# wizardyesterday/RtlSdrDiags

Hardware: NVIDIA B200
Metric: aggregate_iq_msamples_per_s (higher is better)
Workload: dtype q15 int32 + f32

## Files before the change

### rtlsdrdiags_b200/csrc/sdr_device.cuh

```cuda
#pragma once
#include "sdr_platform.h"
#include "sdr_q15_taps.h"

namespace sdr {

enum { FMT_U8_OFFSET_ROTATE = 0, FMT_S8_ROTATED = 1 };
enum { MODE_NONE = 0, MODE_AM = 1, MODE_FM = 2, MODE_WBFM = 3, MODE_LSB = 4, MODE_USB = 5 };

constexpr int MAX_G = 32;
constexpr int FM_LUT_MIN = -140;
constexpr int FM_LUT_DIM = 280;

struct LaunchParams {
  const uint8_t *iq;
  uint64_t ch_stride;
  uint32_t n_samples;
  int fmt;
  const uint32_t *chan_ids;
  uint32_t n_list;
  uint32_t G;
  uint8_t *state;
  uint32_t state_stride;
  const float *scale;
  const uint8_t *lsb;
// ... 2 lines not shown
  const float *lut;
  uint32_t aux;
  int16_t *scratch;
  const uint8_t *allowed;
  uint32_t call_id;
  const uint32_t *tab;
  unsigned long long *trace;
  uint32_t seg_count, seg_rows, warm_rows;
  uint32_t *counters;
};

#if SDR_DEVICE_BUILD
__device__ __forceinline__ unsigned long long trace_now() {
  unsigned long long t;
  asm volatile("mov.u64 %0, %%globaltimer;" : "=l"(t));
  return t;
}
__device__ __forceinline__ void trace_begin(const LaunchParams &p) {
  if (p.trace && threadIdx.x == 0) atomicMin(p.trace, trace_now());
}
__device__ __forceinline__ void trace_end(const LaunchParams &p) {
  if (p.trace && threadIdx.x == 0) atomicMax(p.trace + 1, trace_now());
}
#endif

SDR_DEV int f2i16_wrap(float v) {
  int r = f2i_rz(v);
  if (!(fabsf(v) < 2147483648.0f)) r = 0;
  return (int)(int16_t)(uint16_t)(uint32_t)r;
}

SDR_DEV float wrap_pi(float d) {
  const float PI_F = 3.14159274101257324f;
  const double off = d >= PI_F ? -6.283185307179586 : (d <= -PI_F ? 6.283185307179586 : 0.0);
  return dadd_to_f(d, off);
}

SDR_DEV float wrap_pi_table(float d) {
  const float PI_F = 3.14159274101257324f;
  const float sgn = u2f((f2u(d) & 0x80000000u) | 0x3F800000u);
  const float w = ffma(sgn, u2f(0x343BBD2Eu) ,
                       ffma(sgn, u2f(0xC0C90FDBu) , d));
  return fabsf(d) >= PI_F ? w : d;
}

SDR_DEV uint32_t offset_and_negate(uint32_t raw, uint32_t neg, uint32_t one) {
// ... 203 lines not shown
```

### rtlsdrdiags_b200/csrc/sdr_engine.cu

```cuda
#include <cuda.h>
#include <cuda_runtime.h>
#include <math.h>
#include <stdio.h>
#include <stdlib.h>
#include <string.h>

#include <algorithm>
#include <string>
#include <vector>

#include "../../include/sdr_b200.h"
#include "sdr_config.h"

namespace {

using namespace sdr;

thread_local std::string g_create_error;

struct Shape { uint32_t G = 0, NT = 0; };

}

struct sdr_engine {
  int device = 0;
  uint32_t n = 0;
  uint64_t max_bytes = 0;
  int n_sm = 148;
  int smem_optin = 227 * 1024;
  cudaStream_t own_stream = nullptr, stream = nullptr;
  cudaStream_t rec_stream = nullptr;
  static constexpr int RING_MAX = 3;
  static constexpr int ring = RING_MAX;
  cudaEvent_t ev_fir[RING_MAX] = {}, ev_rec[RING_MAX] = {};
  static constexpr int RUN_AHEAD = 32, PACE = 2 * RUN_AHEAD;
  cudaEvent_t ev_pace[PACE] = {};
  int16_t *d_scratch[5][RING_MAX] = {};
  int tile_loader = 2;
  bool stage1_mma = false;
  int wb_kernel = 0;
  volatile uint32_t *h_wb_clip = nullptr;
  uint32_t wb_clip_seen = 0;
  uint64_t wb4_units = 0;
  int wb_clip_hold = 0;
  int wb4_geometry = 0;
  bool wb_count = false;
  bool wb_prefilter_mma = false;
  int fir_ctas_per_sm = 5;
  uint32_t *d_am_tab = nullptr;
  CUtensorMap tmap;
  const void *tmap_iq = nullptr;
  uint64_t tmap_stride = 0, tmap_rows = 0;
  uint32_t dc_seg_count = 0, dc_warm_rows = 28;
  uint32_t *d_counters = nullptr;
  uint64_t seq = 0;
  bool rec_pending = false;
  cudaStream_t wb_stream = nullptr;
  cudaEvent_t ev_in = nullptr, ev_wb = nullptr;
  bool wb_pending = false;
  int scaling = SDR_SCALING_RADIODIAGS;

  std::vector<uint8_t> mode, lsb;
  std::vector<float> gain[5], scale[5];
  std::vector<uint32_t> list[5];
  bool lists_dirty = true, lsb_dirty = true, scale_dirty[5] = {true, true, true, true, true};

  uint8_t *d_state[5] = {};
  float *d_scale[5] = {};
  uint32_t *d_list[5] = {};
  uint8_t *d_lsb = nullptr;
  float *d_lut_fm = nullptr, *d_lut_wbfm = nullptr;
  float *d_lut_wbfm_half = nullptr;
  uint32_t *d_fm_tab = nullptr;
  uint32_t *d_wb_tab = nullptr;
  uint8_t *d_wb4_tab = nullptr;
  uint8_t *d_iq = nullptr;
  int16_t *d_pcm2[2] = {nullptr, nullptr};
  uint64_t pcm_stride = 0;
  int16_t *pcm_of(uint64_t call) const { return d_pcm2[call & 1]; }
// ... 62 lines not shown
  }
  return 0;
}

float default_gain(int kind, int scaling) {
  switch (kind) {
    case SDR_KIND_AM: return 300;
    case SDR_KIND_FM: return (float)(64000 / (2 * M_PI));
    case SDR_KIND_WBFM:
      return scaling == SDR_SCALING_RESEARCH ? (float)(64000 / (2 * M_PI)) : (float)(256000 / (2 * M_PI));
    case SDR_KIND_SSB: return 300;
  }
  return 0;
}

float scale_of(int kind, float gain, int scaling) {
  if (kind == SDR_KIND_AM || kind == SDR_KIND_SSB || scaling == SDR_SCALING_RESEARCH) return gain;
  volatile float k = gain / (kind == SDR_KIND_FM ? 15000.0f : 75000.0f);
  k = k * 32767.0f;
  return k;
}

int join_streams(sdr_engine *e) {
  if (e->rec_pending) {
    SDR_CK(e, cudaStreamWaitEvent(e->stream, e->ev_rec[(e->seq + (uint64_t)e->ring - 1) % (uint64_t)e->ring], 0));
    e->rec_pending = false;
  }
  if (e->wb_pending) {
    SDR_CK(e, cudaStreamWaitEvent(e->stream, e->ev_wb, 0));
    e->wb_pending = false;
  }
  return SDR_OK;
}

typedef CUresult (*TensorMapEncodeTiled)(CUtensorMap *, CUtensorMapDataType, cuuint32_t, void *, const cuuint64_t *,
                                         const cuuint64_t *, const cuuint32_t *, const cuuint32_t *,
                                         CUtensorMapInterleave, CUtensorMapSwizzle, CUtensorMapL2promotion,
                                         CUtensorMapFloatOOBfill);
int iq_tensor_map(sdr_engine *e, const uint8_t *iq, uint64_t ch_stride, uint32_t n_samples) {
  const uint64_t rows = (uint64_t)(n_samples / TILE) * (TILE_BYTES / 128);
  if (e->tmap_iq == iq && e->tmap_stride == ch_stride && e->tmap_rows == rows) return SDR_OK;
  static TensorMapEncodeTiled encode = nullptr;
  if (!encode) {
    void *fn = nullptr;
    cudaDriverEntryPointQueryResult qr;
    SDR_CK(e, cudaGetDriverEntryPoint("cuTensorMapEncodeTiled", &fn, cudaEnableDefault, &qr));
    if (!fn || qr != cudaDriverEntryPointSuccess) return fail(e, SDR_E_CUDA, "the driver has no cuTensorMapEncodeTiled");
    encode = (TensorMapEncodeTiled)fn;
  }
  if (rows == 0) {
// ... 45 lines not shown
    };
    for (int lane = 0; lane < 32; ++lane) {
      const int g = lane >> 2, tq = lane & 3;
      uint32_t *t = tab.data() + ((size_t)f * 32 + lane) * 12;
      for (int h = 0; h < 2; ++h)
        for (int s2 = 0; s2 < 2; ++s2)
          for (int r = 0; r < 2; ++r) {
            const int k0 = 32 * s2 + 16 * r + 4 * tq;
            uint32_t w = 0;
            for (int b = 0; b < 4; ++b) w |= (uint32_t)(uint8_t)(int8_t)part(B[k0 + b][g], h) << (8 * b);
            t[(h * 2 + s2) * 2 + r] = w;
          }
      for (int i = 0; i < 4; ++i) {
        const int h = i >> 1, col = 2 * tq + (i & 1);
        int sum = 0;
        for (int kb = 0; kb < 64; ++kb) sum += part(B[kb][col], h);
        t[8 + i] = (uint32_t)((h == 1 ? 1 << 15 : 0) - (f == 0 ? 128 * sum : 0));
      }
    }
  }
  return tab;
}

template <bool SSB>
int launch_amssb(sdr_engine *e, int kind, const uint8_t *iq, uint64_t ch_stride, uint32_t n_samples, int fmt) {
  using T = AmSsbTile<SSB>;
  const uint32_t n_list = (uint32_t)e->list[kind].size();
  if (n_list == 0) return SDR_OK;
  const int par = (int)(e->seq % (uint64_t)e->ring);
  const uint32_t n_tiles = (n_samples + TILE - 1) / TILE;
  if (!e->d_scratch[kind][par]) {
    const size_t max_tiles = (size_t)((e->max_bytes / 2 + TILE - 1) / TILE);
    for (int i = 0; i < e->ring; ++i)
      if (!e->d_scratch[kind][i])
        SDR_CK(e, cudaMalloc(&e->d_scratch[kind][i], (size_t)e->n * max_tiles * 32 * sizeof(int16_t)));
  }
  static const int wps_env = getenv("SDR_AM_WARPS_PER_SM") ? atoi(getenv("SDR_AM_WARPS_PER_SM")) : 0;
  const uint64_t total_tiles = (uint64_t)n_list * n_tiles;
  uint64_t n_warps = (uint64_t)e->n_sm * (wps_env > 0 ? wps_env : (SSB ? 48 : 72));
  static const int min_share_env = getenv("SDR_AM_MIN_SHARE") ? atoi(getenv("SDR_AM_MIN_SHARE")) : 0;
  const uint64_t min_share = min_share_env > 0 ? (uint64_t)min_share_env : 16;
  n_warps = std::min<uint64_t>(n_warps, (total_tiles + min_share - 1) / min_share);
  n_warps = std::max<uint64_t>(n_warps, 1);
  LaunchParams p = {};
  p.iq = iq;
  p.ch_stride = ch_stride;
  p.n_samples = n_samples;
  p.fmt = fmt;
  p.chan_ids = e->d_list[kind];
  p.n_list = n_list;
  p.G = 4;
  p.state = e->d_state[kind];
  p.state_stride = (uint32_t)T::STATE_BYTES;
  p.scale = e->d_scale[kind];
  p.lsb = e->d_lsb;
  p.pcm = e->pcm_of(e->seq);
  p.pcm_stride = e->pcm_stride;
  p.lut = nullptr;
  p.aux = (uint32_t)n_warps;
  p.call_id = (uint32_t)(e->seq % 0x7fffffffull) + 1;
  p.scratch = e->d_scratch[kind][par];
  p.allowed = e->last_gated ? e->d_allowed[par] : nullptr;
  p.trace = e->d_trace ? e->d_trace + 4 * (e->seq % sdr_engine::TRACE_CALLS) : nullptr;
  const uint32_t grid = (uint32_t)((n_warps + 3) / 4);
  if (e->tile_loader == 0) {
    if (e->fir_ctas_per_sm == 6) amssb_fir_kernel<SSB, false, 2, false, 6><<<grid, 128, 4 * 2 * TILE_BYTES, e->stream>>>(p, e->tmap);
    else amssb_fir_kernel<SSB, false, 2, false><<<grid, 128, 4 * 2 * TILE_BYTES, e->stream>>>(p, e->tmap);
  } else if (e->fir_ctas_per_sm == 6 && !e->stage1_mma) {
    const int rc = iq_tensor_map(e, iq, ch_stride, n_samples);
    if (rc) return rc;
    if (e->tile_loader == 2) amssb_fir_kernel<SSB, true, 2, false, 6><<<grid, 128, 4 * 2 * TILE_BYTES, e->stream>>>(p, e->tmap);
    else amssb_fir_kernel<SSB, true, 4, false, 6><<<grid, 128, 4 * 4 * TILE_BYTES, e->stream>>>(p, e->tmap);
  } else {
    int rc = iq_tensor_map(e, iq, ch_stride, n_samples);
    if (rc) return rc;
    if (e->stage1_mma && !e->d_am_tab) {
      const std::vector<uint32_t> tab = am_mma_table();
      SDR_CK(e, cudaMalloc(&e->d_am_tab, tab.size() * 4));
      SDR_CK(e, cudaMemcpy(e->d_am_tab, tab.data(), tab.size() * 4, cudaMemcpyHostToDevice));
    }
    p.tab = e->d_am_tab;
    const int nst = e->tile_loader;
    const size_t smem = (size_t)4 * nst * TILE_BYTES;
    if (e->stage1_mma) {
      if (nst == 2) amssb_fir_kernel<SSB, true, 2, true><<<grid, 128, smem, e->stream>>>(p, e->tmap);
      else if (nst == 3) amssb_fir_kernel<SSB, true, 3, true><<<grid, 128, smem, e->stream>>>(p, e->tmap);
      else amssb_fir_kernel<SSB, true, 4, true><<<grid, 128, smem, e->stream>>>(p, e->tmap);
    } else {
      if (nst == 2) amssb_fir_kernel<SSB, true, 2, false><<<grid, 128, smem, e->stream>>>(p, e->tmap);
      else if (nst == 3) amssb_fir_kernel<SSB, true, 3, false><<<grid, 128, smem, e->stream>>>(p, e->tmap);
      else amssb_fir_kernel<SSB, true, 4, false><<<grid, 128, smem, e->stream>>>(p, e->tmap);
    }
  }
  SDR_CK(e, cudaGetLastError());
  e->launches++;
  return SDR_OK;
}

void dc_segments(const sdr_engine *e, uint32_t n_rows, uint32_t *seg_count, uint32_t *seg_rows) {
  uint32_t S = 1;
  if (e->dc_seg_count) {
    S = e->dc_seg_count;
  } else if (n_rows >= 64) {
    while (S < 32 && n_rows / (2 * S) >= 32) S *= 2;
  }
  while (S > 1 && (n_rows + S - 1) / S * (S - 1) >= n_rows) S /= 2;
  *seg_count = S;
  *seg_rows = (n_rows + S - 1) / S;
}

int launch_dc_block(sdr_engine *e, int kind, uint32_t n_samples) {
  const uint32_t n_list = (uint32_t)e->list[kind].size();
  if (n_list == 0) return SDR_OK;
  const int par = (int)(e->seq % (uint64_t)e->ring);
  const int nreg = kind == SDR_KIND_SSB ? AmSsbTile<true>::NREG : AmSsbTile<false>::NREG;
  LaunchParams p = {};
  p.n_samples = n_samples;
  p.chan_ids = e->d_list[kind];
  p.n_list = n_list;
  p.state = e->d_state[kind];
  p.state_stride = (uint32_t)state_bytes(kind);
  p.scale = e->d_scale[kind];
  p.pcm = e->pcm_of(e->seq);
  p.pcm_stride = e->pcm_stride;
  p.aux = (uint32_t)nreg * 256;
  p.scratch = e->d_scratch[kind][par];
  p.allowed = e->last_gated ? e->d_allowed[par] : nullptr;
  p.trace = e->d_trace ? e->d_trace + 4 * (e->seq % sdr_engine::TRACE_CALLS) + 2 : nullptr;
  dc_segments(e, (n_samples + TILE - 1) / TILE, &p.seg_count, &p.seg_rows);
  p.warm_rows = e->dc_warm_rows;
  p.counters = e->d_counters;
  const uint64_t lanes = (uint64_t)n_list * p.seg_count;
  dc_block_kernel<<<(uint32_t)((lanes + 31) / 32), 64, 0, e->rec_stream>>>(p);
  SDR_CK(e, cudaGetLastError());
  e->launches++;
  return SDR_OK;
}

std::vector<uint32_t> fm_mma_table() {
  std::vector<uint32_t> tab(2 * FM_TAB_WORDS_PER_FMT, 0);
  for (int f = 0; f < 2; ++f) {
    int A[16][128] = {};
    for (int kk = 0; kk < 128; ++kk) {
      const int j = (kk - 64) >> 1, c = kk & 1, jm = ((j % 4) + 4) % 4;
      int arm, sign;
      if (f == 0) {
        static const int arm_of[4][2] = {{0, 1}, {1, 0}, {0, 1}, {1, 0}};
        static const int sign_of[4][2] = {{1, 1}, {1, -1}, {-1, -1}, {-1, 1}};
        arm = arm_of[jm][c];
        sign = sign_of[jm][c];
      } else {
        arm = c;
        sign = 1;
      }
      for (int pp = 0; pp < 8; ++pp) {
        const int k = 4 * pp + 3 - j;
        if (k >= 0 && k < taps::FM_TUNER::N) A[8 * arm + pp][kk] = sign * taps::FM_TUNER::tap(k);
      }
    }
// ... 106 lines not shown
  LaunchParams p = {};
  p.iq = iq;
  p.ch_stride = ch_stride;
  p.n_samples = n_samples;
  p.fmt = fmt;
  p.chan_ids = e->d_list[kind];
  p.n_list = n_list;
  p.G = G;
  p.state = e->d_state[kind];
  p.state_stride = (uint32_t)FmTile::STATE_BYTES;
  p.scale = e->d_scale[kind];
  p.lsb = e->d_lsb;
  p.pcm = e->pcm_of(e->seq);
  p.pcm_stride = e->pcm_stride;
  p.lut = e->d_lut_fm;
  p.aux = (uint32_t)n_warps;
  p.call_id = (uint32_t)(e->seq % 0x7fffffffull) + 1;
  p.tab = e->d_fm_tab;
  p.scratch = nullptr;
  p.allowed = e->last_gated ? e->d_allowed[e->seq % (uint64_t)e->ring] : nullptr;
  const uint32_t grid = (uint32_t)((n_warps + G - 1) / G);
  static const int minb_env = getenv("SDR_FM_MIN_CTAS") ? atoi(getenv("SDR_FM_MIN_CTAS")) : 0;
  switch (minb_env) {
    case 5: fm_tile_kernel<5><<<grid, 32 * G, smem, e->stream>>>(p); break;
    case 6: fm_tile_kernel<6><<<grid, 32 * G, smem, e->stream>>>(p); break;
    default: fm_tile_kernel<4><<<grid, 32 * G, smem, e->stream>>>(p); break;
  }
  SDR_CK(e, cudaGetLastError());
  e->launches++;
  return SDR_OK;
}

std::vector<uint8_t> wb_umma_table() {
  std::vector<uint8_t> tab(WB4_TAB_BYTES, 0);
  auto part = [](int v, int h) {
    const int lo = ((v + 128) & 255) - 128;
    return h == 0 ? (v - lo) / 256 : lo;
  };
  for (int kb = 0; kb < 64; ++kb) {
    const int c = kb >> 1, comp = kb & 1, cm = c & 3;
    const int arm = (cm & 1) ? 1 - comp : comp;
    for (int pp = 0; pp < 16; ++pp) {
      const int k = 16 + pp - c;
      if (k < 0 || k >= taps::WB_PRE::N) continue;
      const int v = WbUmma::sign_of(cm, arm) * 2 * taps::WB_PRE::tap(k);
      for (int h = 0; h < 2; ++h)
        tab[((kb >> 5) * 2 + h) * WB4_B_TILE + WbUmma::b_offset(2 * pp + arm, kb & 31)] = (uint8_t)(int8_t)part(v, h);
    }
  }
  return tab;
}

int wb_tab_ready(sdr_engine *e) {
// ... 397 lines not shown
    return fail(nullptr, SDR_E_ARG, "n_channels and max_bytes_per_channel (multiple of 64) must be positive");
  int count = 0;
  cudaError_t ce = cudaGetDeviceCount(&count);
  if (ce != cudaSuccess || count == 0)
    return fail(nullptr, SDR_E_CUDA, "no CUDA device: this engine has no CPU path", ce);
  if (device < 0 || device >= count) return fail(nullptr, SDR_E_ARG, "device index out of range");
  sdr_engine *e = new (std::nothrow) sdr_engine();
  if (!e) return SDR_E_NOMEM;
  e->device = device;
  e->n = n_channels;
  e->max_bytes = max_bytes_per_channel;
#define SDR_CK_CREATE(call)                                                       \
  do {                                                                            \
    cudaError_t _ce = (call);                                                     \
    if (_ce != cudaSuccess) {                                                     \
      fail(nullptr, SDR_E_CUDA, #call, _ce);                                      \
      sdr_engine_destroy(e);                                                      \
      return _ce == cudaErrorMemoryAllocation ? SDR_E_NOMEM : SDR_E_CUDA;         \
    }                                                                             \
  } while (0)
  SDR_CK_CREATE(cudaSetDevice(device));
  SDR_CK_CREATE(cudaDeviceGetAttribute(&e->n_sm, cudaDevAttrMultiProcessorCount, device));
  SDR_CK_CREATE(cudaDeviceGetAttribute(&e->smem_optin, cudaDevAttrMaxSharedMemoryPerBlockOptin, device));
  SDR_CK_CREATE(cudaStreamCreateWithFlags(&e->own_stream, cudaStreamNonBlocking));
  {
    int prio_lo = 0, prio_hi = 0;
    SDR_CK_CREATE(cudaDeviceGetStreamPriorityRange(&prio_lo, &prio_hi));
    SDR_CK_CREATE(cudaStreamCreateWithPriority(&e->rec_stream, cudaStreamNonBlocking, prio_hi));
    SDR_CK_CREATE(cudaStreamCreateWithPriority(&e->wb_stream, cudaStreamNonBlocking, prio_hi));
    SDR_CK_CREATE(cudaEventCreateWithFlags(&e->ev_in, cudaEventDisableTiming));
    SDR_CK_CREATE(cudaEventCreateWithFlags(&e->ev_wb, cudaEventDisableTiming));
  }
  for (int i = 0; i < sdr_engine::RING_MAX; ++i) {
    SDR_CK_CREATE(cudaEventCreateWithFlags(&e->ev_fir[i], cudaEventDisableTiming));
    SDR_CK_CREATE(cudaEventCreateWithFlags(&e->ev_rec[i], cudaEventDisableTiming));
  }
  for (int i = 0; i < sdr_engine::PACE; ++i)
    SDR_CK_CREATE(cudaEventCreateWithFlags(&e->ev_pace[i], cudaEventDisableTiming));
  if (getenv("SDR_TRACE") && atoi(getenv("SDR_TRACE"))) {
    std::vector<unsigned long long> init(4 * sdr_engine::TRACE_CALLS);
    for (size_t i = 0; i < init.size(); ++i) init[i] = (i & 1) ? 0ull : ~0ull;
    SDR_CK_CREATE(cudaMalloc(&e->d_trace, init.size() * 8));
    SDR_CK_CREATE(cudaMemcpy(e->d_trace, init.data(), init.size() * 8, cudaMemcpyHostToDevice));
  }
  SDR_CK_CREATE(cudaMalloc(&e->d_counters, 16));
  SDR_CK_CREATE(cudaMemset(e->d_counters, 0, 16));
  e->stream = e->own_stream;

  e->dump_on.assign(n_channels, 0);
  e->threshold.assign(n_channels, -200);
  e->rx_gain_db.assign(n_channels, 0);
  e->mode.assign(n_channels, SDR_MODE_NONE);
  e->lsb.assign(n_channels, 1);
  for (int k = 1; k <= 4; ++k) {
    e->gain[k].assign(n_channels, default_gain(k, e->scaling));
    e->scale[k].assign(n_channels, 0.f);
    const size_t sb = (size_t)state_bytes(k) * n_channels;
    SDR_CK_CREATE(cudaMalloc(&e->d_state[k], sb));
// ... 30 lines not shown
        const float v = (float)atan2((double)q, (double)i);
        h[(size_t)q * 256 + c] = v;
        if (q <= 127 && v != t[(size_t)(q + 128) * 256 + (i + 128)]) odd = false;
        if (q >= 1) {
          const float n = t[(size_t)(128 - q) * 256 + (i + 128)];
          if (memcmp(&n, &v, 4) == 0 || n != -v) odd = false;
        }
      }
    if (odd) {
      SDR_CK_CREATE(cudaMalloc(&e->d_lut_wbfm_half, h.size() * 4));
      SDR_CK_CREATE(cudaMemcpy(e->d_lut_wbfm_half, h.data(), h.size() * 4, cudaMemcpyHostToDevice));
    }
  }
  SDR_CK_CREATE(cudaStreamSynchronize(e->stream));
#undef SDR_CK_CREATE
  *out = e;
  return SDR_OK;
}

int sdr_engine_destroy(sdr_engine *e) {
  if (!e) return SDR_E_ARG;
  cudaSetDevice(e->device);
  if (e->own_stream) cudaStreamSynchronize(e->own_stream);
  if (e->rec_stream) {
    cudaStreamSynchronize(e->rec_stream);
    cudaStreamDestroy(e->rec_stream);
  }
  if (e->wb_stream) {
    cudaStreamSynchronize(e->wb_stream);
    cudaStreamDestroy(e->wb_stream);
  }
  if (e->ev_in) cudaEventDestroy(e->ev_in);
  if (e->ev_wb) cudaEventDestroy(e->ev_wb);
  for (int i = 0; i < sdr_engine::RING_MAX; ++i) {
    if (e->ev_fir[i]) cudaEventDestroy(e->ev_fir[i]);
    if (e->ev_rec[i]) cudaEventDestroy(e->ev_rec[i]);
  }
  for (int i = 0; i < sdr_engine::PACE; ++i)
    if (e->ev_pace[i]) cudaEventDestroy(e->ev_pace[i]);
  for (int k = 1; k <= 4; ++k) {
    for (int i = 0; i < sdr_engine::RING_MAX; ++i) cudaFree(e->d_scratch[k][i]);
    cudaFree(e->d_state[k]);
    cudaFree(e->d_scale[k]);
    cudaFree(e->d_list[k]);
  }
  cudaFree(e->d_threshold);
  cudaFree(e->d_rx_gain);
  cudaFree(e->d_magnitude);
  cudaFree(e->d_tracking);
  cudaFree(e->d_dump);
  cudaFree(e->d_dump_list);
  for (int i = 0; i < sdr_engine::RING_MAX; ++i) cudaFree(e->d_allowed[i]);
  cudaFree(e->d_db_table);
  cudaFree(e->d_lsb);
  cudaFree(e->d_lut_fm);
  cudaFree(e->d_fm_tab);
  cudaFree(e->d_wb_tab);
  cudaFree(e->d_wb4_tab);
  if (e->h_wb_clip) cudaFreeHost((void *)e->h_wb_clip);
  cudaFree(e->d_am_tab);
  cudaFree(e->d_lut_wbfm);
  cudaFree(e->d_lut_wbfm_half);
  cudaFree(e->d_trace);
  cudaFree(e->d_counters);
  cudaFree(e->d_iq);
  cudaFree(e->d_pcm2[0]);
  cudaFree(e->d_pcm2[1]);
  if (e->own_stream) cudaStreamDestroy(e->own_stream);
  delete e;
  return SDR_OK;
}

int sdr_set_stream(sdr_engine *e, void *cuda_stream) {
  if (!e) return SDR_E_ARG;
  SDR_CK(e, cudaStreamSynchronize(e->stream));
  SDR_CK(e, cudaStreamSynchronize(e->rec_stream));
  SDR_CK(e, cudaStreamSynchronize(e->wb_stream));
  e->rec_pending = false;
  e->wb_pending = false;
  e->stream = cuda_stream ? (cudaStream_t)cuda_stream : e->own_stream;
  return SDR_OK;
}

int sdr_set_scaling(sdr_engine *e, int scaling) {
  if (!e || (scaling != SDR_SCALING_RADIODIAGS && scaling != SDR_SCALING_RESEARCH)) return SDR_E_ARG;
  const float old_def = default_gain(SDR_KIND_WBFM, e->scaling), new_def = default_gain(SDR_KIND_WBFM, scaling);
  for (auto &g : e->gain[SDR_KIND_WBFM])
    if (g == old_def) g = new_def;
  e->scaling = scaling;
  e->scale_dirty[SDR_KIND_FM] = e->scale_dirty[SDR_KIND_WBFM] = true;
  return SDR_OK;
}

int sdr_set_mode(sdr_engine *e, uint32_t ch, int mode) {
  if (!e || ch >= e->n || mode < SDR_MODE_NONE || mode > SDR_MODE_USB) return SDR_E_ARG;
  if (e->mode[ch] != mode) {
    e->mode[ch] = (uint8_t)mode;
    e->lists_dirty = true;
  }
  if (mode == SDR_MODE_LSB && !e->lsb[ch]) { e->lsb[ch] = 1; e->lsb_dirty = true; }
  if (mode == SDR_MODE_USB && e->lsb[ch]) { e->lsb[ch] = 0; e->lsb_dirty = true; }
// ... 152 lines not shown

namespace {
int accept_iq(sdr_engine *e, const void *iq, uint64_t bytes, uint64_t ch_stride, uint32_t flags) {
  if (bytes == 0 || bytes % 64) return fail(e, SDR_E_ARG, "bytes_per_channel must be a positive multiple of 64");
  if (bytes > e->max_bytes) return fail(e, SDR_E_TOO_LONG, "bytes_per_channel exceeds max_bytes_per_channel");
  if (ch_stride < bytes || ch_stride % 16 || ((uintptr_t)iq & 15))
    return fail(e, SDR_E_ARG, "iq pointer and channel_stride must be multiples of 16, stride >= bytes");
  SDR_CK(e, cudaSetDevice(e->device));
  int rc = upload_tables(e);
  if (rc) return rc;
  if (e->wb_pending) {
    SDR_CK(e, cudaStreamWaitEvent(e->stream, e->ev_wb, 0));
    e->wb_pending = false;
  }
  const uint8_t *dev_iq = (const uint8_t *)iq;
  uint64_t dev_stride = ch_stride;
  if (!(flags & SDR_IQ_DEVICE)) {
    if (!e->d_iq) SDR_CK(e, cudaMalloc(&e->d_iq, (size_t)e->n * e->max_bytes));
    SDR_CK(e, cudaMemcpy2DAsync(e->d_iq, bytes, iq, ch_stride, bytes, e->n, cudaMemcpyHostToDevice, e->stream));
    dev_iq = e->d_iq;
    dev_stride = bytes;
  }
  const int slot = (int)((e->seq / 4) % (uint64_t)sdr_engine::PACE);
  if (e->seq % 4 == 0 && e->seq >= (uint64_t)sdr_engine::RUN_AHEAD)
    SDR_CK(e, cudaEventSynchronize(e->ev_pace[(int)(((e->seq - (uint64_t)sdr_engine::RUN_AHEAD) / 4) % (uint64_t)sdr_engine::PACE)]));
  const int fmt = (flags & SDR_IQ_S8_ROTATED) ? FMT_S8_ROTATED : FMT_U8_OFFSET_ROTATE;
  const uint32_t n_samples = (uint32_t)(bytes / 2);
  const bool have_rec = !e->list[SDR_KIND_AM].empty() || !e->list[SDR_KIND_SSB].empty();
  const int par = (int)(e->seq % (uint64_t)e->ring);
  if (have_rec || e->squelch_armed || e->signal_reports || e->squelch_dirty) {
    if (cudaEventQuery(e->ev_rec[par]) != cudaSuccess) {
      (void)cudaGetLastError();
      SDR_CK(e, cudaStreamWaitEvent(e->stream, e->ev_rec[par], 0));
    }
  }
  if ((rc = run_iq_dump(e, dev_iq, dev_stride, bytes, fmt))) return rc;
  if ((rc = run_squelch(e, dev_iq, dev_stride, bytes, fmt))) return rc;
  static const int wb_split_env = getenv("SDR_WB_SPLIT") ? atoi(getenv("SDR_WB_SPLIT")) : 1;
  const bool wb_beside = wb_split_env && !e->list[SDR_KIND_WBFM].empty() &&
                         (have_rec || !e->list[SDR_KIND_FM].empty());
  if (wb_beside) {
    SDR_CK(e, cudaEventRecord(e->ev_in, e->stream));
    SDR_CK(e, cudaStreamWaitEvent(e->wb_stream, e->ev_in, 0));
    if ((rc = launch_wbfm_tile(e, dev_iq, dev_stride, n_samples, fmt, e->wb_stream))) return rc;
    SDR_CK(e, cudaEventRecord(e->ev_wb, e->wb_stream));
    e->wb_pending = true;
  }
  if ((rc = launch_amssb<false>(e, SDR_KIND_AM, dev_iq, dev_stride, n_samples, fmt))) return rc;
  if ((rc = launch_amssb<true>(e, SDR_KIND_SSB, dev_iq, dev_stride, n_samples, fmt))) return rc;
  if (have_rec) {
    SDR_CK(e, cudaEventRecord(e->ev_fir[par], e->stream));
    SDR_CK(e, cudaStreamWaitEvent(e->rec_stream, e->ev_fir[par], 0));
    if ((rc = launch_dc_block(e, SDR_KIND_AM, n_samples))) return rc;
    if ((rc = launch_dc_block(e, SDR_KIND_SSB, n_samples))) return rc;
  }
  SDR_CK(e, cudaEventRecord(e->ev_rec[par], e->rec_stream));
  e->rec_pending = true;
  if ((rc = launch_fm_tile(e, dev_iq, dev_stride, n_samples, fmt))) return rc;
  if (!wb_beside && (rc = launch_wbfm_tile(e, dev_iq, dev_stride, n_samples, fmt, e->stream))) return rc;
  if (e->seq % 4 == 0) SDR_CK(e, cudaEventRecord(e->ev_pace[slot], e->stream));
  e->seq++;
  e->last_samples = (uint32_t)(bytes / 64);
  return SDR_OK;
}
}

extern "C" {

int sdr_get_pcm(sdr_engine *e, int16_t *pcm, uint32_t *counts) {
  if (!e) return SDR_E_ARG;
  if (e->poisoned) return poisoned(e);
  SDR_CK(e, cudaSetDevice(e->device));
  {
    int rc = join_streams(e);
    if (rc) return rc;
  }
  if (pcm && e->last_samples)
    SDR_CK(e, cudaMemcpy2DAsync(pcm, (size_t)e->last_samples * 2, e->pcm_of(e->seq - 1), e->pcm_stride * 2,
                                (size_t)e->last_samples * 2, e->n, cudaMemcpyDeviceToHost, e->stream));
  std::vector<uint8_t> gate;
  if (counts && e->last_gated && e->seq > 0) {
    gate.resize(e->n);
    SDR_CK(e, cudaMemcpyAsync(gate.data(), e->d_allowed[(e->seq + (uint64_t)e->ring - 1) % (uint64_t)e->ring], e->n, cudaMemcpyDeviceToHost, e->stream));
// ... 505 lines not shown
```

### rtlsdrdiags_b200/csrc/sdr_tile.cuh

```cuda
#pragma once
#include "sdr_device.cuh"

#if SDR_DEVICE_BUILD
#include <cuda.h>
#ifndef SDR_FIR_UNROLL
#define SDR_FIR_UNROLL 2
#endif
#ifndef SDR_FM_UNROLL
#define SDR_FM_UNROLL 1
#endif
namespace sdr { constexpr int FIR_UNROLL = SDR_FIR_UNROLL, FM_UNROLL = SDR_FM_UNROLL; }
namespace sdr {

constexpr int TILE = 1024;
constexpr int TILE_BYTES = 2 * TILE;
constexpr unsigned FULL = 0xffffffffu;

template <class T>
__device__ __forceinline__ T shfl_prev(T cur, T prev, int j, int lane) {
  return __shfl_sync(FULL, lane >= 32 - j ? prev : cur, (lane - j) & 31);
}
template <class T>
__device__ __forceinline__ T roll_prev(T cur, T prev, int r, int lane) {
  return __shfl_sync(FULL, lane >= r ? prev : cur, (lane + r) & 31);
// ... 419 lines not shown
  __device__ __forceinline__ static void hilbert_ring(int &h, uint32_t at) {
    if constexpr (K <= 30) {
      int v;
      asm volatile("ld.shared.u32 %0, [%1+%2];" : "=r"(v) : "r"(at), "n"(-4 * K) : "memory");
      h += taps::SSB_HILBERT::tap(K) * v;
      hilbert_ring<K + 2>(h, at);
    }
  }
};

template <bool SSB, bool TMA, int NST, bool MMA, int MINB = 5>
__global__ void __launch_bounds__(128, MINB) amssb_fir_kernel(const __grid_constant__ LaunchParams p,
                                                           const __grid_constant__ CUtensorMap tmap) {
  using T = AmSsbTile<SSB>;
  constexpr uint32_t WARMUP = T::WARMUP_TILES;
  static_assert(!MMA || TMA, "the tensor-core stage 1 reads the TMA slot layout");
  extern __shared__ __align__(1024) uint4 smem_raw[];
  __shared__ uint64_t s_bar[4][NST];
  __shared__ uint4 s_mma[MMA ? 4 : 1][34];
  __shared__ uint32_t s_ring[4][SSB ? 128 : 64];
  const int lane = threadIdx.x & 31, warp = __shfl_sync(FULL, (int)(threadIdx.x >> 5), 0);
  const uint32_t n_warps = p.aux;
  const uint32_t gw = blockIdx.x * (blockDim.x >> 5) + warp;
  trace_begin(p);
  if (gw >= n_warps) return;
  const uint32_t n_tiles = (p.n_samples + TILE - 1) / TILE;
  const uint64_t total = (uint64_t)p.n_list * n_tiles;
  uint64_t g0 = total * gw / n_warps;
  const uint64_t g1 = total * (gw + 1) / n_warps;

  char *slots = reinterpret_cast<char *>(smem_raw) + warp * NST * TILE_BYTES;
  TileIo io;
  TmaIo tio;
  if constexpr (TMA) tio.init(slots, s_bar[warp], lane, NST);
  else io.init(slots, lane);
  const int fmt = p.fmt;
  typename T::Mma mm;
  if constexpr (MMA) {
    const uint32_t ms = (uint32_t)__cvta_generic_to_shared(s_mma[warp]);
    mm.init(p.tab, fmt, ms, ms + 32, lane);
  }

  while (g0 < g1) {
    const uint32_t li = (uint32_t)(g0 / n_tiles);
    const uint32_t t0 = (uint32_t)(g0 - (uint64_t)li * n_tiles);
    const uint32_t t1 = (uint32_t)min((uint64_t)n_tiles, t0 + (g1 - g0));
    g0 += t1 - t0;
    const uint32_t ch = __shfl_sync(FULL, p.chan_ids[li], 0);
    if (p.allowed && !p.allowed[ch]) continue;
    const uint8_t *src = p.iq + (uint64_t)ch * p.ch_stride;
    uint32_t *blob = reinterpret_cast<uint32_t *>(p.state + (uint64_t)ch * p.state_stride);
    const uint32_t tw = t0 <= WARMUP ? 0 : t0 - WARMUP;
    AmSsbCarry<SSB> pv;
    uint32_t *version = blob + T::TAIL_OFFSET / 4 + 2;
    if (tw == 0) {
      const uint32_t v = *reinterpret_cast<volatile uint32_t *>(version);
      const uint32_t cur = (v & 0x7fffffffu) == p.call_id ? (v >> 31) ^ 1u : v >> 31;
      T::load_carry(pv, blob + cur * T::CARRY_WORDS, lane);
    } else {
      pv.a7 = pv.b7 = pv.s1a0 = pv.s1a1 = pv.s1b0 = pv.s1b1 = pv.p = 0;
      pv.dem = 0;
      pv.y3a = pv.y3b = 0;
    }
    const bool lsb = SSB && p.lsb[ch] != 0;
    const uint32_t hring = (uint32_t)__cvta_generic_to_shared(s_ring[warp]);
    T::ring_init(hring, pv, lane);
    bool force_simt = false, planes_ok = true;
    if constexpr (MMA) {
      __syncwarp();
      uint32_t w0, w1;
      T::raw_from_planes(pv.a7, pv.b7, fmt, w0, w1);
      if (lane < 6) asm volatile("st.shared.u32 [%0], %1;" ::"r"(mm.hist_s + 4 * lane), "r"(0x80808080u) : "memory");
      if (lane == 31) asm volatile("st.shared.v2.u32 [%0], {%1,%2};" ::"r"(mm.hist_s + 24), "r"(w0), "r"(w1) : "memory");
      if (fmt == FMT_U8_OFFSET_ROTATE)
        force_simt = __any_sync(FULL, lane == 31 && ((w0 & 0xff000000u) == 0 || (((w1 | 0xff000000u) - 0x01010101u) & ~(w1 | 0xff000000u) & 0x80808080u) != 0));
      __syncwarp();
    }

// ... 54 lines not shown
          __syncwarp();
          io.read(buf * TILE_BYTES, w);
        }
        __syncwarp();
        d = T::template tile<true>(w, fmt, lsb, pv, lane, 32, hring);
      }
      if (t >= t0) *sp = (int16_t)d;
      sp += 32;
      buf = buf + 1 == NST ? 0 : buf + 1;
    }
    if constexpr (MMA) {
      if (!planes_ok) T::planes_from_history(mm.hist_s, fmt, pv);
    }
    if (partial) {
      cp_async_wait<0>();
      __syncwarp();
      uint32_t w[16];
      tile_read(slots + buf * TILE_BYTES, lane, w);
      const int r = (int)(p.n_samples - tf * TILE) >> 5;
      const int d = T::template tile<false>(w, fmt, lsb, pv, lane, r, hring);
      if (lane < r) *sp = (int16_t)d;
    }
    if (t1 == n_tiles) {
      const uint32_t nxt = (*reinterpret_cast<volatile uint32_t *>(version) >> 31) ^ 1u;
      T::store_carry(pv, blob + nxt * T::CARRY_WORDS, lane);
      __syncwarp();
      if (lane == 0) *reinterpret_cast<volatile uint32_t *>(version) = (nxt << 31) | p.call_id;
    }
  }
  if (p.trace && lane == 0) atomicMax(p.trace + 1, trace_now());
}

constexpr int DC_PF = 8;
constexpr int DC_LANE_PITCH = 80;
constexpr int DC_STAGE_BYTES = 32 * DC_LANE_PITCH;
constexpr int DC_Y_PITCH = 144;
constexpr int DC_Y_BYTES = 32 * DC_Y_PITCH;

struct DcRows {
  uint32_t begin, store, end;
};

__device__ __forceinline__ void dc_fetch_row(uint32_t stage_s, const int16_t *g) {
  asm volatile(
      "cp.async.cg.shared.global [%0], [%1], 16;\n\t"
      "cp.async.cg.shared.global [%0+16], [%1+16], 16;\n\t"
      "cp.async.cg.shared.global [%0+32], [%1+32], 16;\n\t"
      "cp.async.cg.shared.global [%0+48], [%1+48], 16;" ::"r"(stage_s), "l"(g)
      : "memory");
}

__global__ void __launch_bounds__(64, 16) dc_block_kernel(const __grid_constant__ LaunchParams p) {
  trace_begin(p);
  const int lane = threadIdx.x & 31;
  const bool chain = threadIdx.x < 32;
  const uint32_t S = p.seg_count, Lr = p.seg_rows;
  const uint32_t idx = blockIdx.x * 32u + (uint32_t)lane;
  const uint32_t li = idx / S, s = idx & (S - 1);
  const uint32_t n_rows = (p.n_samples + TILE - 1) / TILE;
  const uint32_t n_pcm = p.n_samples >> 5;
  const float a1 = (float)(-0.95);

  bool valid = li < p.n_list && s * Lr < n_rows;
  const uint32_t ch = valid ? p.chan_ids[li] : 0;
  if (valid && p.allowed && !p.allowed[ch]) valid = false;
  float *tail = reinterpret_cast<float *>(p.state + (uint64_t)ch * p.state_stride + p.aux);
  const float carried = valid ? tail[1] : 0.f;
  const float gain = valid ? p.scale[ch] : 0.f;
  int16_t *out = p.pcm + (uint64_t)ch * p.pcm_stride;
  const int16_t *src = p.scratch + (uint64_t)(valid ? li : 0) * n_rows * 32;
  const bool no_patch = __all_sync(FULL, !valid || (fabsf(gain) < 500.f && fabsf(carried) < 2e6f));

  __shared__ uint4 s_ring[DC_PF * DC_STAGE_BYTES / 16];
  __shared__ uint4 s_y[2 * DC_Y_BYTES / 16];
  __shared__ uint32_t s_begin[32];
  __shared__ uint32_t s_more;
// ... 394 lines not shown
    if (r == 32) {
#pragma unroll
      for (int i = 0; i < 4; ++i) { pv.th[i] = cu.th[i]; pv.dw[i] = cu.dw[i]; }
      pv.ew = cu.ew;
    } else {
#pragma unroll
      for (int i = 0; i < 4; ++i) {
        pv.th[i] = roll_prev(cu.th[i], pv.th[i], r, lane);
        pv.dw[i] = roll_prev(cu.dw[i], pv.dw[i], r, lane);
      }
      pv.ew = roll_prev(cu.ew, pv.ew, r, lane);
    }
    __syncwarp();
    ering[lane] = pv.ew;
    return pcm;
  }
};

template <int MIN_CTAS>
__global__ void __launch_bounds__(128, MIN_CTAS) fm_tile_kernel(const __grid_constant__ LaunchParams p) {
  extern __shared__ uint4 smem_raw[];
  __shared__ uint4 s_tab[FM_TAB_WORDS_PER_FMT / 4];
  const int lane = threadIdx.x & 31, warp = threadIdx.x >> 5;
  {
    const uint4 *src4 = reinterpret_cast<const uint4 *>(p.tab + (p.fmt == FMT_U8_OFFSET_ROTATE ? 0 : FM_TAB_WORDS_PER_FMT));
    for (int i = threadIdx.x; i < FM_TAB_WORDS_PER_FMT / 4; i += blockDim.x) s_tab[i] = src4[i];
  }
  __syncthreads();
  const uint32_t n_warps = p.aux;
  const uint32_t gw = blockIdx.x * (blockDim.x >> 5) + warp;
  if (gw >= n_warps) return;
  const uint32_t n_tiles = (p.n_samples + TILE - 1) / TILE;
  const uint64_t total = (uint64_t)p.n_list * n_tiles;
  uint64_t g0 = total * gw / n_warps;
  const uint64_t g1 = total * (gw + 1) / n_warps;

  char *wbase = reinterpret_cast<char *>(smem_raw) + warp * FM_WARP_SMEM;
  char *buf0 = wbase + FM_HIST_BYTES;
  float *thbuf = reinterpret_cast<float *>(wbase + 2 * FM_BUF_STRIDE);
  uint32_t *ering = reinterpret_cast<uint32_t *>(wbase + 2 * FM_BUF_STRIDE + 32 * FM_TH_STRIDE * 4);
  TileIo io;
  io.init(buf0, lane);
  const uint32_t buf0_s = (uint32_t)__cvta_generic_to_shared(buf0);
  const int fmt = p.fmt;
  FmTile::Mma mm;
  mm.init(reinterpret_cast<const uint32_t *>(s_tab), lane);
  constexpr uint32_t WARMUP = FmTile::WARMUP_TILES;

  while (g0 < g1) {
    const uint32_t li = (uint32_t)(g0 / n_tiles);
    const uint32_t t0 = (uint32_t)(g0 - (uint64_t)li * n_tiles);
// ... 470 lines not shown
```

Baseline: 2.442 million.

## Replace DC-block side stream with programmatic dependent launch chaining on one stream

Removes the separate high-priority recorder stream and its per-call events, and launches the AM/SSB FIR, DC-block and FM kernels on the main stream with cudaLaunchKernelEx and programmatic stream serialization. Kernels call griddepcontrol.launch_dependents early and griddepcontrol.wait before touching dependent state, so the next kernel's prologue can overlap the previous kernel's tail. A heuristic based on the FIR CTA count versus device thread capacity and the call sequence decides when chaining is allowed, and pacing events are now recorded as programmatic events. This trades the concurrency of two streams for lower launch and inter-kernel gaps, but adds ordering risk because the carry state is read and written around the wait points.

```diff
diff --git a/rtlsdrdiags_b200/csrc/sdr_device.cuh b/rtlsdrdiags_b200/csrc/sdr_device.cuh
--- a/rtlsdrdiags_b200/csrc/sdr_device.cuh
+++ b/rtlsdrdiags_b200/csrc/sdr_device.cuh
@@ -48,6 +48,9 @@
 __device__ __forceinline__ void trace_end(const LaunchParams &p) {
   if (p.trace && threadIdx.x == 0) atomicMax(p.trace + 1, trace_now());
 }
+
+__device__ __forceinline__ void chain_release() { asm volatile("griddepcontrol.launch_dependents;" ::: "memory"); }
+__device__ __forceinline__ void chain_wait() { asm volatile("griddepcontrol.wait;" ::: "memory"); }
 #endif
 
 SDR_DEV int f2i16_wrap(float v) {
diff --git a/rtlsdrdiags_b200/csrc/sdr_engine.cu b/rtlsdrdiags_b200/csrc/sdr_engine.cu
--- a/rtlsdrdiags_b200/csrc/sdr_engine.cu
+++ b/rtlsdrdiags_b200/csrc/sdr_engine.cu
@@ -29,10 +29,12 @@
   int n_sm = 148;
   int smem_optin = 227 * 1024;
   cudaStream_t own_stream = nullptr, stream = nullptr;
-  cudaStream_t rec_stream = nullptr;
   static constexpr int RING_MAX = 3;
   static constexpr int ring = RING_MAX;
-  cudaEvent_t ev_fir[RING_MAX] = {}, ev_rec[RING_MAX] = {};
+  bool chain_open = false;
+  uint32_t fir_ctas[2] = {};
+  int threads_per_sm = 2048;
+  cudaEvent_t pace_due = nullptr;
   static constexpr int RUN_AHEAD = 32, PACE = 2 * RUN_AHEAD;
   cudaEvent_t ev_pace[PACE] = {};
   int16_t *d_scratch[5][RING_MAX] = {};
@@ -54,7 +56,6 @@
   uint32_t dc_seg_count = 0, dc_warm_rows = 28;
   uint32_t *d_counters = nullptr;
   uint64_t seq = 0;
-  bool rec_pending = false;
   cudaStream_t wb_stream = nullptr;
   cudaEvent_t ev_in = nullptr, ev_wb = nullptr;
   bool wb_pending = false;
@@ -163,10 +164,6 @@
 }
 
 int join_streams(sdr_engine *e) {
-  if (e->rec_pending) {
-    SDR_CK(e, cudaStreamWaitEvent(e->stream, e->ev_rec[(e->seq + (uint64_t)e->ring - 1) % (uint64_t)e->ring], 0));
-    e->rec_pending = false;
-  }
   if (e->wb_pending) {
     SDR_CK(e, cudaStreamWaitEvent(e->stream, e->ev_wb, 0));
     e->wb_pending = false;
@@ -258,26 +255,57 @@
   return tab;
 }
 
+template <typename... P, typename... A>
+int launch_chained(sdr_engine *e, void (*kernel)(P...), uint32_t grid, uint32_t block, size_t smem, A &&...args) {
+  cudaLaunchAttribute attr[2];
+  attr[0].id = cudaLaunchAttributeProgrammaticStreamSerialization;
+  attr[0].val.programmaticStreamSerializationAllowed = e->chain_open ? 1 : 0;
+  unsigned n_attr = 1;
+  if (e->pace_due) {
+    attr[1].id = cudaLaunchAttributeProgrammaticEvent;
+    attr[1].val.programmaticEvent.event = e->pace_due;
+    attr[1].val.programmaticEvent.flags = 0;
+    attr[1].val.programmaticEvent.triggerAtBlockStart = 0;
+    n_attr = 2;
+  }
+  cudaLaunchConfig_t cfg = {};
+  cfg.gridDim = dim3(grid);
+  cfg.blockDim = dim3(block);
+  cfg.dynamicSmemBytes = smem;
+  cfg.stream = e->stream;
+  cfg.attrs = attr;
+  cfg.numAttrs = n_attr;
+  SDR_CK(e, cudaLaunchKernelEx(&cfg, kernel, std::forward<A>(args)...));
+  e->chain_open = true;
+  e->pace_due = nullptr;
+  e->launches++;
+  return SDR_OK;
+}
+
+uint64_t amssb_warps(const sdr_engine *e, bool SSB, uint32_t n_samples) {
+  static const int wps_env = getenv("SDR_AM_WARPS_PER_SM") ? atoi(getenv("SDR_AM_WARPS_PER_SM")) : 0;
+  const uint32_t n_tiles = (n_samples + TILE - 1) / TILE;
+  const uint64_t total_tiles = (uint64_t)e->list[SSB ? SDR_KIND_SSB : SDR_KIND_AM].size() * n_tiles;
+  uint64_t n_warps = (uint64_t)e->n_sm * (wps_env > 0 ? wps_env : (SSB ? 48 : 72));
+  static const int min_share_env = getenv("SDR_AM_MIN_SHARE") ? atoi(getenv("SDR_AM_MIN_SHARE")) : 0;
+  const uint64_t min_share = min_share_env > 0 ? (uint64_t)min_share_env : 16;
+  n_warps = std::min<uint64_t>(n_warps, (total_tiles + min_share - 1) / min_share);
+  return std::max<uint64_t>(n_warps, 1);
+}
+
 template <bool SSB>
 int launch_amssb(sdr_engine *e, int kind, const uint8_t *iq, uint64_t ch_stride, uint32_t n_samples, int fmt) {
   using T = AmSsbTile<SSB>;
   const uint32_t n_list = (uint32_t)e->list[kind].size();
   if (n_list == 0) return SDR_OK;
   const int par = (int)(e->seq % (uint64_t)e->ring);
-  const uint32_t n_tiles = (n_samples + TILE - 1) / TILE;
   if (!e->d_scratch[kind][par]) {
     const size_t max_tiles = (size_t)((e->max_bytes / 2 + TILE - 1) / TILE);
     for (int i = 0; i < e->ring; ++i)
       if (!e->d_scratch[kind][i])
         SDR_CK(e, cudaMalloc(&e->d_scratch[kind][i], (size_t)e->n * max_tiles * 32 * sizeof(int16_t)));
   }
-  static const int wps_env = getenv("SDR_AM_WARPS_PER_SM") ? atoi(getenv("SDR_AM_WARPS_PER_SM")) : 0;
-  const uint64_t total_tiles = (uint64_t)n_list * n_tiles;
-  uint64_t n_warps = (uint64_t)e->n_sm * (wps_env > 0 ? wps_env : (SSB ? 48 : 72));
-  static const int min_share_env = getenv("SDR_AM_MIN_SHARE") ? atoi(getenv("SDR_AM_MIN_SHARE")) : 0;
-  const uint64_t min_share = min_share_env > 0 ? (uint64_t)min_share_env : 16;
-  n_warps = std::min<uint64_t>(n_warps, (total_tiles + min_share - 1) / min_share);
-  n_warps = std::max<uint64_t>(n_warps, 1);
+  const uint64_t n_warps = amssb_warps(e, SSB, n_samples);
   LaunchParams p = {};
   p.iq = iq;
   p.ch_stride = ch_stride;
@@ -299,17 +327,17 @@
   p.allowed = e->last_gated ? e->d_allowed[par] : nullptr;
   p.trace = e->d_trace ? e->d_trace + 4 * (e->seq % sdr_engine::TRACE_CALLS) : nullptr;
   const uint32_t grid = (uint32_t)((n_warps + 3) / 4);
+  e->fir_ctas[0] += grid;
+  int rc = SDR_OK;
   if (e->tile_loader == 0) {
-    if (e->fir_ctas_per_sm == 6) amssb_fir_kernel<SSB, false, 2, false, 6><<<grid, 128, 4 * 2 * TILE_BYTES, e->stream>>>(p, e->tmap);
-    else amssb_fir_kernel<SSB, false, 2, false><<<grid, 128, 4 * 2 * TILE_BYTES, e->stream>>>(p, e->tmap);
+    if (e->fir_ctas_per_sm == 6) rc = launch_chained(e, amssb_fir_kernel<SSB, false, 2, false, 6>, grid, 128, 4 * 2 * TILE_BYTES, p, e->tmap);
+    else rc = launch_chained(e, amssb_fir_kernel<SSB, false, 2, false>, grid, 128, 4 * 2 * TILE_BYTES, p, e->tmap);
   } else if (e->fir_ctas_per_sm == 6 && !e->stage1_mma) {
-    const int rc = iq_tensor_map(e, iq, ch_stride, n_samples);
-    if (rc) return rc;
-    if (e->tile_loader == 2) amssb_fir_kernel<SSB, true, 2, false, 6><<<grid, 128, 4 * 2 * TILE_BYTES, e->stream>>>(p, e->tmap);
-    else amssb_fir_kernel<SSB, true, 4, false, 6><<<grid, 128, 4 * 4 * TILE_BYTES, e->stream>>>(p, e->tmap);
+    if ((rc = iq_tensor_map(e, iq, ch_stride, n_samples))) return rc;
+    if (e->tile_loader == 2) rc = launch_chained(e, amssb_fir_kernel<SSB, true, 2, false, 6>, grid, 128, 4 * 2 * TILE_BYTES, p, e->tmap);
+    else rc = launch_chained(e, amssb_fir_kernel<SSB, true, 4, false, 6>, grid, 128, 4 * 4 * TILE_BYTES, p, e->tmap);
   } else {
-    int rc = iq_tensor_map(e, iq, ch_stride, n_samples);
-    if (rc) return rc;
+    if ((rc = iq_tensor_map(e, iq, ch_stride, n_samples))) return rc;
     if (e->stage1_mma && !e->d_am_tab) {
       const std::vector<uint32_t> tab = am_mma_table();
       SDR_CK(e, cudaMalloc(&e->d_am_tab, tab.size() * 4));
@@ -319,18 +347,16 @@
     const int nst = e->tile_loader;
     const size_t smem = (size_t)4 * nst * TILE_BYTES;
     if (e->stage1_mma) {
-      if (nst == 2) amssb_fir_kernel<SSB, true, 2, true><<<grid, 128, smem, e->stream>>>(p, e->tmap);
-      else if (nst == 3) amssb_fir_kernel<SSB, true, 3, true><<<grid, 128, smem, e->stream>>>(p, e->tmap);
-      else amssb_fir_kernel<SSB, true, 4, true><<<grid, 128, smem, e->stream>>>(p, e->tmap);
+      if (nst == 2) rc = launch_chained(e, amssb_fir_kernel<SSB, true, 2, true>, grid, 128, smem, p, e->tmap);
+      else if (nst == 3) rc = launch_chained(e, amssb_fir_kernel<SSB, true, 3, true>, grid, 128, smem, p, e->tmap);
+      else rc = launch_chained(e, amssb_fir_kernel<SSB, true, 4, true>, grid, 128, smem, p, e->tmap);
     } else {
-      if (nst == 2) amssb_fir_kernel<SSB, true, 2, false><<<grid, 128, smem, e->stream>>>(p, e->tmap);
-      else if (nst == 3) amssb_fir_kernel<SSB, true, 3, false><<<grid, 128, smem, e->stream>>>(p, e->tmap);
-      else amssb_fir_kernel<SSB, true, 4, false><<<grid, 128, smem, e->stream>>>(p, e->tmap);
-    }
-  }
-  SDR_CK(e, cudaGetLastError());
-  e->launches++;
-  return SDR_OK;
+      if (nst == 2) rc = launch_chained(e, amssb_fir_kernel<SSB, true, 2, false>, grid, 128, smem, p, e->tmap);
+      else if (nst == 3) rc = launch_chained(e, amssb_fir_kernel<SSB, true, 3, false>, grid, 128, smem, p, e->tmap);
+      else rc = launch_chained(e, amssb_fir_kernel<SSB, true, 4, false>, grid, 128, smem, p, e->tmap);
+    }
+  }
+  return rc;
 }
 
 void dc_segments(const sdr_engine *e, uint32_t n_rows, uint32_t *seg_count, uint32_t *seg_rows) {
@@ -367,10 +393,7 @@
   p.warm_rows = e->dc_warm_rows;
   p.counters = e->d_counters;
   const uint64_t lanes = (uint64_t)n_list * p.seg_count;
-  dc_block_kernel<<<(uint32_t)((lanes + 31) / 32), 64, 0, e->rec_stream>>>(p);
-  SDR_CK(e, cudaGetLastError());
-  e->launches++;
-  return SDR_OK;
+  return launch_chained(e, dc_block_kernel, (uint32_t)((lanes + 31) / 32), 64, 0, p);
 }
 
 std::vector<uint32_t> fm_mma_table() {
@@ -523,13 +546,10 @@
   const uint32_t grid = (uint32_t)((n_warps + G - 1) / G);
   static const int minb_env = getenv("SDR_FM_MIN_CTAS") ? atoi(getenv("SDR_FM_MIN_CTAS")) : 0;
   switch (minb_env) {
-    case 5: fm_tile_kernel<5><<<grid, 32 * G, smem, e->stream>>>(p); break;
-    case 6: fm_tile_kernel<6><<<grid, 32 * G, smem, e->stream>>>(p); break;
-    default: fm_tile_kernel<4><<<grid, 32 * G, smem, e->stream>>>(p); break;
-  }
-  SDR_CK(e, cudaGetLastError());
-  e->launches++;
-  return SDR_OK;
+    case 5: return launch_chained(e, fm_tile_kernel<5>, grid, 32 * G, smem, p);
+    case 6: return launch_chained(e, fm_tile_kernel<6>, grid, 32 * G, smem, p);
+    default: return launch_chained(e, fm_tile_kernel<4>, grid, 32 * G, smem, p);
+  }
 }
 
 std::vector<uint8_t> wb_umma_table() {
@@ -973,18 +993,14 @@
   SDR_CK_CREATE(cudaSetDevice(device));
   SDR_CK_CREATE(cudaDeviceGetAttribute(&e->n_sm, cudaDevAttrMultiProcessorCount, device));
   SDR_CK_CREATE(cudaDeviceGetAttribute(&e->smem_optin, cudaDevAttrMaxSharedMemoryPerBlockOptin, device));
+  SDR_CK_CREATE(cudaDeviceGetAttribute(&e->threads_per_sm, cudaDevAttrMaxThreadsPerMultiProcessor, device));
   SDR_CK_CREATE(cudaStreamCreateWithFlags(&e->own_stream, cudaStreamNonBlocking));
   {
     int prio_lo = 0, prio_hi = 0;
     SDR_CK_CREATE(cudaDeviceGetStreamPriorityRange(&prio_lo, &prio_hi));
-    SDR_CK_CREATE(cudaStreamCreateWithPriority(&e->rec_stream, cudaStreamNonBlocking, prio_hi));
     SDR_CK_CREATE(cudaStreamCreateWithPriority(&e->wb_stream, cudaStreamNonBlocking, prio_hi));
     SDR_CK_CREATE(cudaEventCreateWithFlags(&e->ev_in, cudaEventDisableTiming));
     SDR_CK_CREATE(cudaEventCreateWithFlags(&e->ev_wb, cudaEventDisableTiming));
-  }
-  for (int i = 0; i < sdr_engine::RING_MAX; ++i) {
-    SDR_CK_CREATE(cudaEventCreateWithFlags(&e->ev_fir[i], cudaEventDisableTiming));
-    SDR_CK_CREATE(cudaEventCreateWithFlags(&e->ev_rec[i], cudaEventDisableTiming));
   }
   for (int i = 0; i < sdr_engine::PACE; ++i)
     SDR_CK_CREATE(cudaEventCreateWithFlags(&e->ev_pace[i], cudaEventDisableTiming));
@@ -1061,20 +1077,12 @@
   if (!e) return SDR_E_ARG;
   cudaSetDevice(e->device);
   if (e->own_stream) cudaStreamSynchronize(e->own_stream);
-  if (e->rec_stream) {
-    cudaStreamSynchronize(e->rec_stream);
-    cudaStreamDestroy(e->rec_stream);
-  }
   if (e->wb_stream) {
     cudaStreamSynchronize(e->wb_stream);
     cudaStreamDestroy(e->wb_stream);
   }
   if (e->ev_in) cudaEventDestroy(e->ev_in);
   if (e->ev_wb) cudaEventDestroy(e->ev_wb);
-  for (int i = 0; i < sdr_engine::RING_MAX; ++i) {
-    if (e->ev_fir[i]) cudaEventDestroy(e->ev_fir[i]);
-    if (e->ev_rec[i]) cudaEventDestroy(e->ev_rec[i]);
-  }
   for (int i = 0; i < sdr_engine::PACE; ++i)
     if (e->ev_pace[i]) cudaEventDestroy(e->ev_pace[i]);
   for (int k = 1; k <= 4; ++k) {
@@ -1113,9 +1121,7 @@
 int sdr_set_stream(sdr_engine *e, void *cuda_stream) {
   if (!e) return SDR_E_ARG;
   SDR_CK(e, cudaStreamSynchronize(e->stream));
-  SDR_CK(e, cudaStreamSynchronize(e->rec_stream));
   SDR_CK(e, cudaStreamSynchronize(e->wb_stream));
-  e->rec_pending = false;
   e->wb_pending = false;
   e->stream = cuda_stream ? (cudaStream_t)cuda_stream : e->own_stream;
   return SDR_OK;
@@ -1314,18 +1320,16 @@
     dev_stride = bytes;
   }
   const int slot = (int)((e->seq / 4) % (uint64_t)sdr_engine::PACE);
+  if (e->seq % 4 == 0) e->pace_due = e->ev_pace[slot];
   if (e->seq % 4 == 0 && e->seq >= (uint64_t)sdr_engine::RUN_AHEAD)
     SDR_CK(e, cudaEventSynchronize(e->ev_pace[(int)(((e->seq - (uint64_t)sdr_engine::RUN_AHEAD) / 4) % (uint64_t)sdr_engine::PACE)]));
   const int fmt = (flags & SDR_IQ_S8_ROTATED) ? FMT_S8_ROTATED : FMT_U8_OFFSET_ROTATE;
   const uint32_t n_samples = (uint32_t)(bytes / 2);
   const bool have_rec = !e->list[SDR_KIND_AM].empty() || !e->list[SDR_KIND_SSB].empty();
-  const int par = (int)(e->seq % (uint64_t)e->ring);
-  if (have_rec || e->squelch_armed || e->signal_reports || e->squelch_dirty) {
-    if (cudaEventQuery(e->ev_rec[par]) != cudaSuccess) {
-      (void)cudaGetLastError();
-      SDR_CK(e, cudaStreamWaitEvent(e->stream, e->ev_rec[par], 0));
-    }
-  }
+  const uint64_t fir_threads = 128ull * (e->fir_ctas[0] + e->fir_ctas[1]);
+  e->chain_open = !have_rec || fir_threads > (uint64_t)e->n_sm * (uint64_t)e->threads_per_sm || e->seq % 3 != 0;
+  e->fir_ctas[1] = e->fir_ctas[0];
+  e->fir_ctas[0] = 0;
   if ((rc = run_iq_dump(e, dev_iq, dev_stride, bytes, fmt))) return rc;
   if ((rc = run_squelch(e, dev_iq, dev_stride, bytes, fmt))) return rc;
   static const int wb_split_env = getenv("SDR_WB_SPLIT") ? atoi(getenv("SDR_WB_SPLIT")) : 1;
@@ -1340,17 +1344,14 @@
   }
   if ((rc = launch_amssb<false>(e, SDR_KIND_AM, dev_iq, dev_stride, n_samples, fmt))) return rc;
   if ((rc = launch_amssb<true>(e, SDR_KIND_SSB, dev_iq, dev_stride, n_samples, fmt))) return rc;
-  if (have_rec) {
-    SDR_CK(e, cudaEventRecord(e->ev_fir[par], e->stream));
-    SDR_CK(e, cudaStreamWaitEvent(e->rec_stream, e->ev_fir[par], 0));
-    if ((rc = launch_dc_block(e, SDR_KIND_AM, n_samples))) return rc;
-    if ((rc = launch_dc_block(e, SDR_KIND_SSB, n_samples))) return rc;
-  }
-  SDR_CK(e, cudaEventRecord(e->ev_rec[par], e->rec_stream));
-  e->rec_pending = true;
+  if ((rc = launch_dc_block(e, SDR_KIND_AM, n_samples))) return rc;
+  if ((rc = launch_dc_block(e, SDR_KIND_SSB, n_samples))) return rc;
   if ((rc = launch_fm_tile(e, dev_iq, dev_stride, n_samples, fmt))) return rc;
   if (!wb_beside && (rc = launch_wbfm_tile(e, dev_iq, dev_stride, n_samples, fmt, e->stream))) return rc;
-  if (e->seq % 4 == 0) SDR_CK(e, cudaEventRecord(e->ev_pace[slot], e->stream));
+  if (e->pace_due) {
+    SDR_CK(e, cudaEventRecord(e->pace_due, e->stream));
+    e->pace_due = nullptr;
+  }
   e->seq++;
   e->last_samples = (uint32_t)(bytes / 64);
   return SDR_OK;
diff --git a/rtlsdrdiags_b200/csrc/sdr_tile.cuh b/rtlsdrdiags_b200/csrc/sdr_tile.cuh
--- a/rtlsdrdiags_b200/csrc/sdr_tile.cuh
+++ b/rtlsdrdiags_b200/csrc/sdr_tile.cuh
@@ -465,8 +465,12 @@
   const int lane = threadIdx.x & 31, warp = __shfl_sync(FULL, (int)(threadIdx.x >> 5), 0);
   const uint32_t n_warps = p.aux;
   const uint32_t gw = blockIdx.x * (blockDim.x >> 5) + warp;
+  chain_release();
   trace_begin(p);
-  if (gw >= n_warps) return;
+  if (gw >= n_warps) {
+    chain_wait();
+    return;
+  }
   const uint32_t n_tiles = (p.n_samples + TILE - 1) / TILE;
   const uint64_t total = (uint64_t)p.n_list * n_tiles;
   uint64_t g0 = total * gw / n_warps;
@@ -497,6 +501,7 @@
     AmSsbCarry<SSB> pv;
     uint32_t *version = blob + T::TAIL_OFFSET / 4 + 2;
     if (tw == 0) {
+      chain_wait();
       const uint32_t v = *reinterpret_cast<volatile uint32_t *>(version);
       const uint32_t cur = (v & 0x7fffffffu) == p.call_id ? (v >> 31) ^ 1u : v >> 31;
       T::load_carry(pv, blob + cur * T::CARRY_WORDS, lane);
@@ -597,12 +602,14 @@
       if (lane < r) *sp = (int16_t)d;
     }
     if (t1 == n_tiles) {
+      chain_wait();
       const uint32_t nxt = (*reinterpret_cast<volatile uint32_t *>(version) >> 31) ^ 1u;
       T::store_carry(pv, blob + nxt * T::CARRY_WORDS, lane);
       __syncwarp();
       if (lane == 0) *reinterpret_cast<volatile uint32_t *>(version) = (nxt << 31) | p.call_id;
     }
   }
+  chain_wait();
   if (p.trace && lane == 0) atomicMax(p.trace + 1, trace_now());
 }
 
@@ -626,7 +633,9 @@
 }
 
 __global__ void __launch_bounds__(64, 16) dc_block_kernel(const __grid_constant__ LaunchParams p) {
+  chain_release();
   trace_begin(p);
+  chain_wait();
   const int lane = threadIdx.x & 31;
   const bool chain = threadIdx.x < 32;
   const uint32_t S = p.seg_count, Lr = p.seg_rows;
@@ -1067,11 +1076,13 @@
   extern __shared__ uint4 smem_raw[];
   __shared__ uint4 s_tab[FM_TAB_WORDS_PER_FMT / 4];
   const int lane = threadIdx.x & 31, warp = threadIdx.x >> 5;
+  chain_release();
   {
     const uint4 *src4 = reinterpret_cast<const uint4 *>(p.tab + (p.fmt == FMT_U8_OFFSET_ROTATE ? 0 : FM_TAB_WORDS_PER_FMT));
     for (int i = threadIdx.x; i < FM_TAB_WORDS_PER_FMT / 4; i += blockDim.x) s_tab[i] = src4[i];
   }
   __syncthreads();
+  chain_wait();
   const uint32_t n_warps = p.aux;
   const uint32_t gw = blockIdx.x * (blockDim.x >> 5) + warp;
   if (gw >= n_warps) return;
```

Result: slower. 1.950 million, median of 6 (-20.1%).
